# shacklettbp/madrona-learn

Hardware: AMD Instinct MI355X
Metric: env-steps/sec whole-node, 65536-env PPO, at 1/2/4/8 MI355X (higher is better)
Workload: dtype bf16; 1 GPU; 65536-env PPO iteration (BASELINE metric; SURVEY B8 semantics): T=32, obs=64, MLP[256,256], heads [4,8,5,5,2,2]+critic, 2 epochs x 32 minibatches of 2048 seqs (global), envs and minibatches split over 1 GPU(s); config=headline, total_envs=65536, envs_per_gpu=65536, global_minibatch_seqs=2048, minibatches_per_epoch=32, steps_per_update=32, parallelism=dp1, critic=scalar, hip_graph=True, sim_step=whole_rollout_one_launch

## Files before the change

### madrona-learn_amd/csrc/ppo_rows16.h

```cpp

#pragma once


template <int D> __device__ inline float r16_pair_dpp(float a, float b) {
    float r;
    if constexpr (D == 8)
        asm volatile(
            "s_nop 1\n\t"
            "v_add_f32_dpp %0, %1, %1 row_ror:8 row_mask:0xf bank_mask:0x3\n\t"
            "v_add_f32_dpp %0, %2, %2 row_ror:8 row_mask:0xf bank_mask:0xc"
            : "=&v"(r)
            : "v"(a), "v"(b));
    else
        asm volatile(
            "s_nop 1\n\t"
            "v_add_f32_dpp %0, %1, %1 row_ror:12 row_mask:0xf bank_mask:0x5\n\t"
            "v_add_f32_dpp %0, %2, %2 row_ror:4 row_mask:0xf bank_mask:0xa"
            : "=&v"(r)
            : "v"(a), "v"(b));
    return r;
}

__device__ inline int r16_colf(int qd, int lane) {
    const int r = lane & 15, g = lane >> 4;
    return 16 * (4 * qd + (r >> 2)) + 4 * g + (r & 3);
}
__device__ inline void r16_put_cols(float* cpl, const float (&cb)[4], const float (&cg)[4],
                                    int lane) {
#pragma unroll
    for (int qd = 0; qd < 4; ++qd) {
        const int f = r16_colf(qd, lane);
        cpl[f] = cb[qd];
        cpl[kR16H + f] = cg[qd];
    }
}

__device__ inline float r16_rowsum8(const float (&w)[8], int lane) {
    float x[4], y[2];
#pragma unroll
    for (int i = 0; i < 4; ++i) x[i] = r16_pair_dpp<4>(w[i], w[i + 4]);
    const bool h1 = (lane & 2) != 0, h0 = (lane & 1) != 0;
#pragma unroll
    for (int i = 0; i < 2; ++i) {
        const float keep = h1 ? x[i + 2] : x[i], send = h1 ? x[i] : x[i + 2];
        y[i] = keep + xlane<2>(send);
    }
    const float keep = h0 ? y[1] : y[0], send = h0 ? y[0] : y[1];
    return keep + xlane<1>(send);
}

__device__ inline float r16_dy(float z, float mean, float rstd, float gam, float bet, float da,
                               bool live, float& xh) {
    const float zc = z - mean;
    xh = zc * rstd;
    const float y = __builtin_fmaf(zc, rstd * gam, bet);
    return ((y > relu_thr<bf16>()) & live) ? da : 0.f;
}

__device__ inline void r16_dz_block(const f32x4& u, uint32_t (&zwb)[2], float mean,
                                    float rstd, float ca, float cbc, uint32_t (&dzb)[2]) {
#pragma unroll
    for (int k = 0; k < 2; ++k) {
        zwb[k] = r16_late(zwb[k]);
        const f2v zc = up_bf16(zwb[k]) - f2v{mean, mean};
        const f2v d = f2v{rstd, rstd} * f2v{u[2 * k], u[2 * k + 1]} +
                      (f2v{ca, ca} * zc + f2v{cbc, cbc});
        dzb[k] = pk_bf16(d.x, d.y);
    }
}

__device__ inline void r16_ln_bwd(f32x4 (&acc)[kR16NB], uint32_t (&zw)[kR16NB][2],
                                  float mean, float rstd, const float* gm, int g, int lane,
                                  bool live, uint32_t (&dzw)[kR16NB][2], float (&cb)[4],
                                  float (&cg)[4]) {
    mean = r16_late(mean);
    rstd = r16_late(rstd);
    float su = 0.f, sv = 0.f;
    constexpr int ord[4] = {0, 2, 1, 3};
    R16GB gb(gm, g, 0);
#pragma unroll
    for (int qd = 0; qd < kR16NB / 4; ++qd) {
        float wb[8], wg[8];
#pragma unroll
        for (int hp = 0; hp < 2; ++hp) {
            float pb[8], pg[8];
#pragma unroll
            for (int k = 0; k < 2; ++k) {
                const int step = 4 * qd + 2 * hp + k;
                const int b = 4 * qd + ord[2 * hp + k];
                float4 G, B;
                gb.take_now(b, G, B);
                const float gv[4] = {G.x, G.y, G.z, G.w}, bv[4] = {B.x, B.y, B.z, B.w};
                zw[b][0] = r16_late(zw[b][0]);
                zw[b][1] = r16_late(zw[b][1]);
#pragma unroll
                for (int i = 0; i < 4; ++i) {
                    float xh;
                    const float z = up_bf16(zw[b][i >> 1])[i & 1];
                    const float dy = r16_dy(z, mean, rstd, gv[i], bv[i], acc[b][i], live, xh);
                    const float u = dy * gv[i];
                    su += u;
                    sv = __builtin_fmaf(u, xh, sv);
                    acc[b][i] = u;
                    pb[4 * k + i] = dy;
                    pg[4 * k + i] = dy * xh;
                }
            }
            __builtin_amdgcn_sched_barrier(0);
#pragma unroll
            for (int i = 0; i < 4; ++i) {
                wb[4 * hp + i] = r16_pair_dpp<8>(pb[i], pb[4 + i]);
                wg[4 * hp + i] = r16_pair_dpp<8>(pg[i], pg[4 + i]);
            }
        }
        cb[qd] = r16_rowsum8(wb, lane);
        cg[qd] = r16_rowsum8(wg, lane);
    }
    su = add_xor32(add_xor16(su));
    sv = add_xor32(add_xor16(sv));
    const float invH = 1.0f / (float)kR16H;
    const float ca = -(rstd * rstd) * (sv * invH), cbc = -rstd * (su * invH);
#pragma unroll
    for (int b = 0; b < kR16NB; ++b) r16_dz_block(acc[b], zw[b], mean, rstd, ca, cbc, dzw[b]);
}

#ifdef ML_STAMPS
#define R16_STAMP(i) (r16_st[i] = __builtin_amdgcn_s_memtime())
#define R16_STAMPS_OUT()                                                              \
    do {                                                                              \
        if (ws.stamps && (tid & 63) == 0)                                             \
            for (int i_ = 0; i_ < 13; ++i_)                                           \
                ws.stamps[((int64_t)ptile * NT + tt) * 16 + i_] = r16_st[i_];        \
    } while (0)
#else
#define R16_STAMP(i) \
    do {             \
    } while (0)
#define R16_STAMPS_OUT() \
    do {                 \
    } while (0)
#endif

template <bool METRICS, int NW, int NT, int HC>
__global__ __launch_bounds__(64 * NW) __attribute__((amdgpu_waves_per_eu((NW + 3) / 4, (NW + 3) / 4))) void ppo_rows16_kernel(
    PolicyK P, RolloutK ro, const int32_t* __restrict__ mb_seq, int mb, int64_t M,
    const float* __restrict__ adv_st, HpK hp, WsK ws, R16Div dv) {
    extern __shared__ __attribute__((aligned(16))) char smem[];
#ifdef ML_STAMPS
    const uint64_t r16_t_entry = __builtin_amdgcn_s_memtime();
#endif
    typedef R16Lay<HC> LY;
    constexpr int LGS = LY::LGS, NHB = HC / 16;
    char* w1img = smem + LY::OffW1;
    char* whimg = smem + LY::OffWh;
    float* gb = (float*)(smem + LY::OffGb);
    float* hb = (float*)(smem + LY::OffHb);
    const float* bins = (const float*)(smem + LY::OffBins);
    const int tid = threadIdx.x;
    const int wave = __builtin_amdgcn_readfirstlane(tid >> 6);
    bf16* lgs = (bf16*)(smem + LY::OffLg) + wave * 16 * LGS;
    const int K = P.K;
    constexpr int D = kR16D, DS = D / 32;

    {
        static_assert(NW == kR16Waves, "r16_stage stages with kR16Waves waves");
        r16_stage<HC>(P, smem, tid);
        int* tab = (int*)(smem + LY::OffTab);
        if (tid <= MLEARN_MAX_GROUPS) {
            tab[tid] = P.off[tid];
            ((float*)tab)[MLEARN_MAX_GROUPS + 1 + tid] = tid < MLEARN_MAX_GROUPS ? hp.ecoef[tid] : 0.f;
            ((float*)tab)[2 * (MLEARN_MAX_GROUPS + 1) + tid] =
                tid < MLEARN_MAX_GROUPS ? hp.objw[tid] : 0.f;
        }
    }
    __syncthreads();
#ifdef ML_STAMPS
    const uint64_t r16_t_pro = __builtin_amdgcn_s_memtime();
#endif
    const int* t_off = (const int*)(smem + LY::OffTab);
    const float* t_ec = (const float*)t_off + MLEARN_MAX_GROUPS + 1;
    const float* t_ow = t_ec + MLEARN_MAX_GROUPS + 1;

    const int ptile = (int)blockIdx.x * NW + wave;
    const float as0 = adv_st[0], as1 = adv_st[1];
    VnVals vn{hp.norm_vals != 0, {0.f, 0.f, 0.f, 0.f}};
    if (hp.norm_vals)
        for (int i = 0; i < 4; ++i) vn.v[i] = adv_st[2 + i];
    LossAcc m;
    bool did = false;
    uint32_t dz0w[kR16NB][2];
    float cb0[4], cg0[4];
    float* prev_cp = nullptr;
    int64_t prev_row = -1;
    const int ntask = 16 * (K + 1);
    auto slot_of = [&](int64_t rw, uint32_t& tl) {
        const uint32_t f = (uint32_t)rw;
        tl = r16_udiv(f, dv.mb_mag, dv.mb_sh);
        return f - tl * (uint32_t)mb;
    };
    auto srow_of = [&](int64_t rw, uint32_t seq) -> int64_t {
        uint32_t tl;
        (void)slot_of(rw, tl);
        const uint32_t c = r16_udiv(seq, dv.n_mag, dv.n_sh), b = seq - c * (uint32_t)ro.N;
        return rw < M ? ((int64_t)c * ro.bptt + tl) * ro.ld + b : 0;
    };
    int64_t sr_n;
    {
        uint32_t tl;
        const int64_t rw = (int64_t)ptile * (16 * NT) + (tid & 15);
        sr_n = srow_of(rw, (uint32_t)mb_seq[slot_of(rw, tl)]);
    }

#pragma clang loop unroll(disable)
    for (int tt = 0; tt < NT; ++tt) {
#ifdef ML_STAMPS
        uint64_t r16_st[13];
#endif
        R16_STAMP(0);
        const int lane = r16_late(tid & 63), r = lane & 15, g = lane >> 4;
        const int64_t row0 = (int64_t)ptile * (16 * NT) + 16 * tt;
        const int64_t row = row0 + r;
        const bool live = row < M;
        const int64_t sr = sr_n;
        uint32_t seq_n = 0;
        if (tt + 1 < NT) {
            uint32_t tl;
            seq_n = (uint32_t)mb_seq[slot_of(row + 16, tl)];
        }
        bf16x8 xf[DS];
        const bf16* orow = (const bf16*)ro.obs + sr * D;
#pragma unroll
        for (int s = 0; s < DS; ++s)
            xf[s] = *(const bf16x8*)(orow + 32 * s + 8 * g);
        auto lda0 = [&](int ln) {
            const bf16* w0 = (const bf16*)P.wt[0];
            const int rr = ln & 15, gg = ln >> 4;
            return [=](int b, int s) {
                const int n = 16 * b + rr;
                const int64_t idx = ((int64_t)(((n >> 5) * (D >> 4) + 2 * s + (gg >> 1)) * 64 +
                                               (n & 31) + 32 * (gg & 1))) * 8;
                return *(const bf16x8*)(w0 + idx);
            };
        };
        const bool has_ret = ro.ret != nullptr, has_val = ro.values != nullptr;
        float t_adv = ro.adv[sr];
        float rv = (has_ret ? ro.ret : ro.adv)[sr], vv = (has_val ? ro.values : ro.adv)[sr];
        int ract[2];
        float rlp[2];
#pragma unroll
        for (int u = 0; u < 2; ++u) {
            const int grp = (lane + 64 * u) >> 4;
            const int ga = grp < K ? grp : K - 1;
            ract[u] = ro.actions[sr * K + ga];
            rlp[u] = ro.logp[sr * K + ga];
        }
        auto bf0 = [&](int s) { return xf[s]; };
        uint32_t zw0[kR16NB][2], zw[kR16NB][2], aw[kR16NB][2];
        float mean0, rstd0, mean, rstd;
        r16_fwd_layer<DS, kR16Ring0>(lda0(r16_late(lane)), bf0, zw0, mean0, rstd0);
        sr_n = srow_of(row + 16, r16_late(seq_n));
        uint32_t t_a[2];
        float t_b[2];
        {
            t_adv = r16_late(t_adv);
            rv = r16_late(rv);
            vv = r16_late(vv);
            const float retv = has_ret ? rv : t_adv + vv;
            const float ov = has_val ? vv : 0.f;
#pragma unroll
            for (int u = 0; u < 2; ++u) {
                const int grp = (lane + 64 * u) >> 4;
                t_a[u] = grp < K ? (uint32_t)r16_late(ract[u]) : __builtin_bit_cast(uint32_t, retv);
                t_b[u] = grp < K ? r16_late(rlp[u]) : ov;
            }
        }
        R16_STAMP(1);
#ifndef ML_PROBE_NO_X0
        {
            bf16* xrow = (bf16*)ws.x0 + r16_late(row) * D;
#pragma unroll
            for (int s = 0; s < DS; ++s)
                r16_st16(xrow + 32 * s + 8 * g, __builtin_bit_cast(u4r, xf[s]));
        }
#endif
        if (tt > 0) {
            r16_store_rows((bf16*)ws.dz[0] + r16_late(prev_row) * kR16H, dz0w, g);
            r16_put_cols(prev_cp, cb0, cg0, lane);
        }
        r16_ln_apply(zw0, mean0, rstd0, gb, g, aw);
        R16_STAMP(2);
        r16_fwd_layer<kR16KS, kR16Ring>(
            [&](int b, int s) { return r16_row_frag(w1img, 16 * b + r, s, g); },
            [&](int s) { return r16_bfrag(aw, s); }, zw, mean, rstd);
        R16_STAMP(3);
        if (NW > 4 && tt == 0 && wave >= NW / 2) __builtin_amdgcn_s_setprio(1);
#ifndef ML_PROBE_NO_A0
        r16_store_rows((bf16*)ws.a[0] + r16_late(row) * kR16H, aw, g);
#endif
        r16_ln_apply(zw, mean, rstd, gb + 2 * kR16H, g, aw);
        R16_STAMP(4);
        f32x4 ha[NHB];
#pragma unroll
        for (int j = 0; j < NHB; ++j) ha[j] = f32x4{0.f, 0.f, 0.f, 0.f};
        if constexpr (HC == 32) {
            r16_mm<NHB, kR16KS, 4>(
                ha, [&](int j, int s) { return r16_row_frag(whimg, 16 * j + r, s, g); },
                [&](int s) { return r16_bfrag(aw, s); });
        } else {
            const bf16* ht = (const bf16*)P.head_t;
            const uint32_t lo = r16_late((uint32_t)((r + 32 * (g & 1)) * 8 + 4 * (g >> 1)));
            r16_mm<NHB, kR16KS, kR16RingH>(
                ha,
                [&](int j, int s) {
                    const bf16* p = ht + ((j >> 1) * 8192 + s * 1024 + (j & 1) * 128);
                    const u2r a = *(const u2r*)(p + lo);
                    const u2r b = *(const u2r*)(p + 512 + lo);
                    return __builtin_bit_cast(bf16x8, u4r{a[0], a[1], b[0], b[1]});
                },
                [&](int s) { return r16_bfrag(aw, s); });
        }
        r16_store_rows((bf16*)ws.a[1] + r16_late(row) * kR16H, aw, g);
        {
            bf16* lr = lgs + r * LGS;
#pragma unroll
            for (int cbk = 0; cbk < NHB; ++cbk) {
                const int c0 = 16 * cbk + 4 * g;
                float v[4];
#pragma unroll
                for (int i = 0; i < 4; ++i) v[i] = rnd<bf16>(rnd<bf16>(ha[cbk][i]) + rnd<bf16>(hb[c0 + i]));
                *(u2r*)(lr + c0) = u2r{pk_bf16(v[0], v[1]), pk_bf16(v[2], v[3])};
            }
        }
        wave_lds_sync();
        R16_STAMP(5);
        auto loss_task = [&](int task, int act, float olp, float adv, float ret, float oval) {
            const int rr = task & 15, grp = task >> 4;
            bf16* lr = lgs + rr * LGS;
            if (row0 + rr >= M) {
                if (grp < K)
                    for (int j = t_off[grp]; j < t_off[grp + 1]; ++j) lr[j] = (bf16)0.f;
                else if (HC == 32)
                    for (int j = P.A; j < HC; ++j) lr[j] = (bf16)0.f;
                return;
            }
            if (grp < K) {
                if (hp.norm_adv) adv = (adv - as0) * as1;
                const int o0 = t_off[grp];
                loss_group(hp, lr + o0, t_off[grp + 1] - o0, act, olp, adv, t_ec[grp], t_ow[grp],
                           m);
            } else if (HC == 32) {
                loss_value(hp, lr, P.A, HC, ret, oval, m, vn);
            }
        };
        {
#pragma clang loop unroll(disable)
            for (int task = lane, u = 0; task < ntask; task += 64, ++u) {
                did = true;
                const uint32_t a = u == 0 ? t_a[0] : t_a[1];
                const float b = u == 0 ? t_b[0] : t_b[1];
                loss_task(task, (int)a, b, t_adv, __builtin_bit_cast(float, a), b);
            }
        }
        if constexpr (HC != 32) {
            wave_lds_sync();
            const uint32_t rbits = __shfl(K >= 4 ? t_a[1] : t_a[0], (16 * K + r) & 63);
            bf16* lr = lgs + r * LGS;
            const int CB = P.CB;
            if (row0 + r < M) {
                float mean;
                const float R = __builtin_bit_cast(float, rbits);
                const float vl = r16_twohot_ce(lr + P.A, CB, R, bins,
                                               hp.vcoef * hp.inv_s * hp.loss_scale, g, &mean);
                if (g == 0) {
                    const float verr = fabsf(mean - R);
                    m.svl += vl;
                    m.qvl += vl * vl;
                    m.mnvl = fminf(m.mnvl, vl);
                    m.mxvl = fmaxf(m.mxvl, vl);
                    m.serr += verr;
                    m.qerr += verr * verr;
                    m.mnerr = fminf(m.mnerr, verr);
                    m.mxerr = fmaxf(m.mxerr, verr);
                }
            } else {
                for (int j = P.A + g; j < P.A + CB; j += 4) lr[j] = (bf16)0.f;
            }
            for (int j = P.A + CB + g; j < HC; j += 4) lr[j] = (bf16)0.f;
        }
        wave_lds_sync();
        R16_STAMP(6);
        constexpr int HKS = HC / 32;
        bf16x8 dh[HKS];
#pragma unroll
        for (int s2 = 0; s2 < HKS; ++s2) {
            dh[s2] = *(const bf16x8*)(lgs + r * LGS + 32 * s2 + 8 * g);
            r16_st16((bf16*)ws.dhead + r16_late(row) * HC + 32 * s2 + 8 * g,
                     __builtin_bit_cast(u4r, dh[s2]));
        }
        float* cprow = ws.colpart + ((int64_t)ptile * NT + tt) * ws.CP;
#pragma unroll
        for (int c0 = 0; c0 < HC; c0 += 64) {
            if (c0 + lane < HC) {
                float hbs = 0.f;
#pragma unroll
                for (int rr = 0; rr < 16; ++rr) hbs += to_f32(lgs[rr * LGS + c0 + lane]);
                cprow[2 * 2 * kR16H + c0 + lane] = hbs;
            }
        }
        R16_STAMP(7);
        uint32_t dzw[kR16NB][2];
        {
            f32x4 hacc[kR16NB];
#pragma unroll
            for (int b = 0; b < kR16NB; ++b) hacc[b] = f32x4{0.f, 0.f, 0.f, 0.f};
            if constexpr (HC == 32) {
                r16_mm<kR16NB, 1, kR16Ring>(
                    hacc,
                    [&](int b, int) { return r16_tr_frag(whimg, 8 * g, 8 * g + 4, b, lane); },
                    [&](int) { return dh[0]; });
            } else {
                const bf16* hd = (const bf16*)P.head;
                const uint32_t lo = r16_late((uint32_t)((g >> 1) * 512 + (r + 32 * (g & 1)) * 8));
                r16_mm<kR16NB, HKS, kR16RingH>(
                    hacc,
                    [&](int b, int s2) {
                        const bf16* p = hd + ((b >> 1) * (HC / 16) * 512 + s2 * 1024 + (b & 1) * 128);
                        return *(const bf16x8*)(p + lo);
                    },
                    [&](int s2) { return dh[s2]; });
            }
            float cb1[4], cg1[4];
            r16_ln_bwd(hacc, zw, mean, rstd, gb + 2 * kR16H, g, lane, live, dzw, cb1, cg1);
            r16_put_cols(cprow + 2 * kR16H, cb1, cg1, lane);
        }
        r16_store_rows_keep((bf16*)ws.dz[1] + r16_late(row) * kR16H, dzw, g);
        R16_STAMP(8);
        f32x4 acc[kR16NB];
#pragma unroll
        for (int b = 0; b < kR16NB; ++b) acc[b] = f32x4{0.f, 0.f, 0.f, 0.f};
        r16_mm_bm<kR16NB, kR16KS, kR16Ring>(
            acc,
            [&](int b, int s) {
                return r16_tr_frag(w1img, 32 * s + 4 * g, 32 * s + 16 + 4 * g, b, lane);
            },
            [&](int s) { return r16_bfrag(dzw, s); });
        R16_STAMP(9);
        R16_STAMP(10);
        R16_STAMP(11);
        r16_ln_bwd(acc, zw0, mean0, rstd0, gb, g, lane, live, dz0w, cb0, cg0);
        prev_row = row;
        prev_cp = cprow;
        R16_STAMP(12);
        R16_STAMPS_OUT();
    }
    const int lane = tid & 63, r = lane & 15, g = lane >> 4;
    r16_store_rows((bf16*)ws.dz[0] + prev_row * kR16H, dz0w, g);
    r16_put_cols(prev_cp, cb0, cg0, lane);

#ifdef ML_STAMPS
    {
        __builtin_amdgcn_s_waitcnt(0);
        const uint64_t t_end = __builtin_amdgcn_s_memtime();
        if (ws.stamps && (tid & 63) == 0) {
            uint64_t* st = ws.stamps + (int64_t)ptile * NT * 16;
            st[13] = r16_t_entry;
            st[14] = r16_t_pro;
            st[15] = t_end;
        }
    }
#endif
    if (METRICS) {
        const float vals[kLossSlots] = {m.sobj, m.qobj, m.mnobj, m.mxobj, m.svl, m.qvl, m.mnvl,
                                        m.mxvl, m.serr, m.qerr, m.mnerr, m.mxerr, m.sent, m.qent,
                                        m.mnent, m.mxent, m.sentw, m.sobjw, 0.f, 0.f};
        constexpr int kUsed = 18;
        double* lp = ws.loss_part + (int64_t)ptile * kLossSlots;
        if (__any(did)) {
#pragma unroll
            for (int s = 0; s < kUsed; ++s) {
                const int kind = (s < 16) ? (s & 3) : 0;
                float v = vals[s];
                v = kind == 2 ? wave_reduce<2>(v) : (kind == 3 ? wave_reduce<3>(v) : wave_reduce<0>(v));
                if (lane == 0) lp[s] = v;
            }
            if (lane >= kUsed && lane < kLossSlots) lp[lane] = 0.0;
        } else if (lane < kLossSlots) {
            const int kind = (lane < 16) ? (lane & 3) : 0;
            lp[lane] = kind == 2 ? 3.4e38 : (kind == 3 ? -3.4e38 : 0.0);
        }
    }
}

struct R16Cfg {
    int nw, nt;
};
static R16Cfg rows16_cfg(int64_t Mp) {
    const int cus = device_cus();
    const int64_t kCUs = cus > 0 ? cus : 256;
    if (Mp % 256 == 0 && Mp / 256 >= kCUs) return R16Cfg{8, 2};
    if (Mp == 128 * kCUs) return R16Cfg{8, 1};
    return R16Cfg{0, 0};
}
static bool rows16_eligible(const PolicyK& P, int64_t Mp, int HC, int L, int H, bool bf) {
    const bool head = (HC == 32 && P.CB == 1) || (HC == 96 && P.CB > 1 && P.CB <= 64);
    return bf && H == kR16H && L == 2 && head && P.D == kR16D && P.K + 1 <= 8 &&
           rows16_cfg(Mp).nw > 0;
}

template <int NW, int NT, int HC>
static void launch_rows16_cfg(const PolicyK& P, const RolloutK& R, const int32_t* mb_seq, int mb,
                              int64_t M, const float* adv_st, const HpK& hp, const WsK& ws,
                              const R16Div& dv, hipStream_t s) {
    constexpr int lds = (int)R16Lay<HC>::Lds;
    if (set_lds_attr((const void*)ppo_rows16_kernel<true, NW, NT, HC>, lds, "ppo_rows16") ||
        set_lds_attr((const void*)ppo_rows16_kernel<false, NW, NT, HC>, lds, "ppo_rows16"))
        return;
    const int grid = (int)(ws.Mp / (16 * NW * NT));
    if (hp.metrics)
        hipLaunchKernelGGL((ppo_rows16_kernel<true, NW, NT, HC>), dim3(grid), dim3(64 * NW), lds,
                           s, P, R, mb_seq, mb, M, adv_st, hp, ws, dv);
    else
        hipLaunchKernelGGL((ppo_rows16_kernel<false, NW, NT, HC>), dim3(grid), dim3(64 * NW), lds,
                           s, P, R, mb_seq, mb, M, adv_st, hp, ws, dv);
}

static void launch_rows16(const PolicyK& P, const RolloutK& R, const int32_t* mb_seq, int mb,
                          int64_t M, const float* adv_st, const HpK& hp, const WsK& ws,
                          hipStream_t s) {
    R16Div dv;
    r16_magic((uint32_t)mb, dv.mb_mag, dv.mb_sh);
    r16_magic((uint32_t)R.N, dv.n_mag, dv.n_sh);
    const R16Cfg c = rows16_cfg(ws.Mp);
    if (P.HC == 32) {
        if (c.nt == 2)
            launch_rows16_cfg<8, 2, 32>(P, R, mb_seq, mb, M, adv_st, hp, ws, dv, s);
        else
            launch_rows16_cfg<8, 1, 32>(P, R, mb_seq, mb, M, adv_st, hp, ws, dv, s);
    } else {
        if (c.nt == 2)
            launch_rows16_cfg<8, 2, 96>(P, R, mb_seq, mb, M, adv_st, hp, ws, dv, s);
        else
            launch_rows16_cfg<8, 1, 96>(P, R, mb_seq, mb, M, adv_st, hp, ws, dv, s);
    }
}
```

### madrona-learn_amd/csrc/r16_common.h

```cpp
#pragma once

#include "common.h"
#include "dists.h"
#include "rowtile.h"

namespace ml {

constexpr int kR16Waves = 8;
constexpr int kR16Tiles = 2;
constexpr int kR16H = 256;
constexpr int kR16NB = kR16H / 16;
constexpr int kR16KS = kR16H / 32;
constexpr int kR16HC = MLEARN_HEAD_COLS;
constexpr int kR16D = 64;
constexpr int kR16LGS = 40;
#ifndef ML_R16_RING
#define ML_R16_RING 6
#endif
#ifndef ML_R16_RING0
#define ML_R16_RING0 16
#endif
constexpr int kR16Ring = ML_R16_RING;
constexpr int kR16Ring0 = ML_R16_RING0;
#ifndef ML_R16_RINGH
#define ML_R16_RINGH 8
#endif
constexpr int kR16RingH = ML_R16_RINGH;
constexpr int kR16TabN = 3 * (MLEARN_MAX_GROUPS + 1);
template <int HC> struct R16Lay {
    static_assert(HC == 32 || HC == 96, "head width");
    static constexpr int LGS = HC == 32 ? kR16LGS : 104;
    static constexpr size_t OffW1 = 0;
    static constexpr size_t OffWh = OffW1 + (size_t)kR16H * 512;
    static constexpr size_t OffGb = OffWh + (HC == 32 ? (size_t)HC * 512 : 0);
    static constexpr size_t OffHb = OffGb + (size_t)2 * 2 * kR16H * 4;
    static constexpr size_t OffBins = OffHb + (size_t)HC * 4;
    static constexpr size_t OffLg = OffBins + (HC == 32 ? 0 : (size_t)64 * 4);
    static constexpr size_t OffTab = OffLg + (size_t)kR16Waves * 16 * LGS * 2;
    static constexpr size_t Lds = OffTab + (size_t)kR16TabN * 4;
    static_assert(Lds <= 160 * 1024, "row-split LDS budget");
};

typedef float f2v __attribute__((ext_vector_type(2)));
typedef short short4r __attribute__((ext_vector_type(4)));
typedef __attribute__((ext_vector_type(4))) uint32_t u4r;
typedef __attribute__((ext_vector_type(2))) uint32_t u2r;

__device__ inline uint32_t r16_off(int n, int u) {
    const int sw = ((n & 7) << 2) | (((n >> 3) & 1) << 1);
    return (uint32_t)(n * 512 + ((u ^ sw) << 3));
}

template <typename V> __device__ inline V r16_late(V v) {
    asm volatile("" : "+v"(v));
    return v;
}

__device__ inline f32x4 mma16(bf16x8 a, bf16x8 b, f32x4 c) {
    return __builtin_amdgcn_mfma_f32_16x16x32_bf16(a, b, c, 0, 0, 0);
}

__device__ inline bf16x8 r16_row_frag(const char* img, int n, int s, int g) {
    const u2r lo = *(const u2r*)(img + r16_off(n, 8 * s + g));
    const u2r hi = *(const u2r*)(img + r16_off(n, 8 * s + 4 + g));
    const u4r v = {lo[0], lo[1], hi[0], hi[1]};
    return __builtin_bit_cast(bf16x8, v);
}

__device__ inline bf16x8 r16_tr_frag(const char* img, int rlo, int rhi, int b, int lane) {
    const int q = (lane >> 2) & 3, p = lane & 3;
    typedef __attribute__((address_space(3))) short4r* lp;
    const short4r lo = __builtin_amdgcn_ds_read_tr16_b64_v4i16(
        (lp)(img + (rlo & ~15) * 512 + r16_off((rlo & 15) + q, 4 * b + p)));
    const short4r hi = __builtin_amdgcn_ds_read_tr16_b64_v4i16(
        (lp)(img + (rhi & ~15) * 512 + r16_off((rhi & 15) + q, 4 * b + p)));
    typedef short short8r __attribute__((ext_vector_type(8)));
    const short8r v = {lo[0], lo[1], lo[2], lo[3], hi[0], hi[1], hi[2], hi[3]};
    return __builtin_bit_cast(bf16x8, v);
}

__device__ inline void r16_st16(void* p, u4r v) { *(u4r*)p = v; }

__device__ inline uint32_t pk_bf16(float a, float b) {
    typedef __bf16 bf16x2 __attribute__((ext_vector_type(2)));
    const bf16x2 v = {(bf16)a, (bf16)b};
    return __builtin_bit_cast(uint32_t, v);
}
__device__ inline f2v up_bf16(uint32_t w) {
    return f2v{__builtin_bit_cast(float, w << 16), __builtin_bit_cast(float, w & 0xffff0000u)};
}
__device__ inline bf16x8 r16_bfrag(const uint32_t (&w)[kR16NB][2], int s) {
    const u4r v = {w[2 * s][0], w[2 * s][1], w[2 * s + 1][0], w[2 * s + 1][1]};
    return __builtin_bit_cast(bf16x8, v);
}

template <int NBO, int NS, int RING, typename LDA, typename BF>
__device__ inline void r16_mm(f32x4 (&acc)[NBO], LDA lda, BF bfrag) {
    constexpr int N = NS * NBO;
    constexpr int RG = RING < N ? RING : N;
    __builtin_amdgcn_sched_barrier(0);
    bf16x8 ra[RG];
#pragma unroll
    for (int i = 0; i < RG; ++i) ra[i] = lda(i % NBO, i / NBO);
    bf16x8 bfr = bfrag(0);
#pragma unroll
    for (int i = 0; i < N; ++i) {
        const bf16x8 a = ra[i % RG];
        if (i + RG < N) ra[i % RG] = lda((i + RG) % NBO, (i + RG) / NBO);
        __builtin_amdgcn_sched_barrier(0);
        acc[i % NBO] = mma16(a, bfr, acc[i % NBO]);
        __builtin_amdgcn_sched_barrier(0);
        if ((i + 1) % NBO == 0 && i + 1 < N) bfr = bfrag((i + 1) / NBO);
    }
}

template <int NBO, int NS, int RING, typename LDA, typename BF>
__device__ inline void r16_mm_bm(f32x4 (&acc)[NBO], LDA lda, BF bfrag) {
    static_assert(NBO % 2 == 0, "block pairs");
    constexpr int N = NS * NBO;
    constexpr int RG = RING < N ? RING : N;
    auto jof = [](int i) { return 2 * (i / (2 * NS)) + (i & 1); };
    auto sof = [](int i) { return (i >> 1) % NS; };
    __builtin_amdgcn_sched_barrier(0);
    bf16x8 ra[RG];
#pragma unroll
    for (int i = 0; i < RG; ++i) ra[i] = lda(jof(i), sof(i));
#pragma unroll
    for (int i = 0; i < N; ++i) {
        const bf16x8 a = ra[i % RG];
        if (i + RG < N) ra[i % RG] = lda(jof(i + RG), sof(i + RG));
        __builtin_amdgcn_sched_barrier(0);
        acc[jof(i)] = mma16(a, bfrag(sof(i)), acc[jof(i)]);
        __builtin_amdgcn_sched_barrier(0);
    }
}

template <int NS, int RING, typename LDA, typename BF>
__device__ inline void r16_fwd_layer(LDA lda, BF bfrag, uint32_t (&zw)[kR16NB][2], float& mean_o,
                                     float& rstd_o) {
    f2v s2 = {0.f, 0.f}, q2 = {0.f, 0.f};
#pragma unroll
    for (int h = 0; h < 2; ++h) {
        f32x4 acc[8];
#pragma unroll
        for (int j = 0; j < 8; ++j) acc[j] = f32x4{0.f, 0.f, 0.f, 0.f};
        r16_mm<8, NS, RING>(acc, [&](int j, int s) { return lda(8 * h + j, s); }, bfrag);
#pragma unroll
        for (int j = 0; j < 8; ++j)
#pragma unroll
            for (int k = 0; k < 2; ++k) {
                zw[8 * h + j][k] = pk_bf16(acc[j][2 * k], acc[j][2 * k + 1]);
                const f2v x = up_bf16(zw[8 * h + j][k]);
                s2 += x;
                q2 = x * x + q2;
            }
    }
    float sum = s2.x + s2.y, sq = q2.x + q2.y;
    sum = add_xor32(add_xor16(sum));
    sq = add_xor32(add_xor16(sq));
    const float invH = 1.0f / (float)kR16H;
    const float mean = sum * invH;
    const float var = fmaxf(sq * invH - mean * mean, 0.f);
    mean_o = mean;
    rstd_o = rsqrtf(var + 1e-6f);
}

__device__ inline void r16_store_rows(bf16* rowp, uint32_t (&w)[kR16NB][2], int g) {
#pragma unroll
    for (int c = 0; c < kR16NB / 2; ++c) {
#pragma unroll
        for (int k = 0; k < 2; ++k) {
            const auto v = __builtin_amdgcn_permlane16_swap(w[2 * c][k], w[2 * c + 1][k], false,
                                                            false);
            w[2 * c][k] = v[0];
            w[2 * c + 1][k] = v[1];
        }
        const int blk = 2 * c + (g & 1);
        r16_st16(rowp + 16 * blk + 8 * (g >> 1),
                 u4r{w[2 * c][0], w[2 * c][1], w[2 * c + 1][0], w[2 * c + 1][1]});
    }
}

__device__ inline void r16_store_rows_keep(bf16* rowp, const uint32_t (&w)[kR16NB][2], int g) {
#pragma unroll
    for (int c = 0; c < kR16NB / 2; ++c) {
        uint32_t t[2][2];
#pragma unroll
        for (int k = 0; k < 2; ++k) {
            const auto v = __builtin_amdgcn_permlane16_swap(w[2 * c][k], w[2 * c + 1][k], false,
                                                            false);
            t[0][k] = v[0];
            t[1][k] = v[1];
        }
        const int blk = 2 * c + (g & 1);
        r16_st16(rowp + 16 * blk + 8 * (g >> 1), u4r{t[0][0], t[0][1], t[1][0], t[1][1]});
    }
}

struct R16GB {
    const float* gm;
    int g;
    float4 G, B;
    __device__ R16GB(const float* gm_, int g_, int first) : gm(gm_), g(g_) { load(first); }
    __device__ void load(int b) {
        const int f0 = r16_late(16 * b + 4 * g);
        G = *(const float4*)(gm + f0);
        B = *(const float4*)(gm + kR16H + f0);
    }
    __device__ void take_now(int b, float4& Go, float4& Bo) {
        __builtin_amdgcn_sched_barrier(0);
        load(b);
        Go = G;
        Bo = B;
    }
    __device__ void take(int following, float4& Go, float4& Bo) {
        __builtin_amdgcn_sched_barrier(0);
        Go = G;
        Bo = B;
        if (following >= 0) load(following);
    }
};

__device__ inline void r16_ln_apply(uint32_t (&zw)[kR16NB][2], float mean, float rstd,
                                    const float* gm, int g, uint32_t (&aw)[kR16NB][2]) {
    const f2v m2 = {mean, mean}, r2 = {rstd, rstd};
    R16GB gb(gm, g, 0);
#pragma unroll
    for (int b = 0; b < kR16NB; ++b) {
        float4 G, B;
        gb.take(b + 1 < kR16NB ? b + 1 : -1, G, B);
        zw[b][0] = r16_late(zw[b][0]);
        zw[b][1] = r16_late(zw[b][1]);
        const f2v y0 = __builtin_elementwise_fma(up_bf16(zw[b][0]) - m2, r2 * f2v{G.x, G.y},
                                                 f2v{B.x, B.y});
        const f2v y1 = __builtin_elementwise_fma(up_bf16(zw[b][1]) - m2, r2 * f2v{G.z, G.w},
                                                 f2v{B.z, B.w});
        aw[b][0] = pk_bf16(fmaxf(y0.x, 0.f), fmaxf(y0.y, 0.f));
        aw[b][1] = pk_bf16(fmaxf(y1.x, 0.f), fmaxf(y1.y, 0.f));
    }
}

struct R16Div {
    uint32_t mb_mag, n_mag;
    int mb_sh, n_sh;
};
__device__ inline uint32_t r16_udiv(uint32_t n, uint32_t mag, int sh) {
    return (__umulhi(n, mag) + n) >> sh;
}


template <int HC = kR16HC>
__device__ inline void r16_stage(const PolicyK& P, char* smem, int tid) {
    typedef R16Lay<HC> LY;
    char* w1img = smem + LY::OffW1;
    char* whimg = smem + LY::OffWh;
    float* gb = (float*)(smem + LY::OffGb);
    float* hb = (float*)(smem + LY::OffHb);
    {
        const u4r* src1 = (const u4r*)P.wt[1];
        const u4r* srch = (const u4r*)P.head_t;
        constexpr int N1 = kR16H * kR16H * 2 / 16 / (64 * kR16Waves);
        u4r v1[N1], vh[2];
#pragma unroll
        for (int i = 0; i < N1; ++i) v1[i] = src1[tid + i * 64 * kR16Waves];
        if (HC == 32)
#pragma unroll
            for (int i = 0; i < 2; ++i) vh[i] = srch[tid + i * 64 * kR16Waves];
        float pv[2];
#pragma unroll
        for (int i = 0; i < 2; ++i) {
            const int j = tid + i * 64 * kR16Waves, l = j >> 9, c = j & 511;
            pv[i] = c < kR16H ? P.lns[l][c] : P.lnb[l][c - kR16H];
        }
        const float hbv = tid < HC ? P.head_b[tid] : 0.f;
        auto put = [&](char* img, int U, u4r v) {
            const int n = ((U >> 10) << 5) | (U & 31), h = (U >> 5) & 1, s16 = (U >> 6) & 15;
            *(u2r*)(img + r16_off(n, 4 * s16 + h)) = u2r{v[0], v[1]};
            *(u2r*)(img + r16_off(n, 4 * s16 + 2 + h)) = u2r{v[2], v[3]};
        };
#pragma unroll
        for (int i = 0; i < N1; ++i) put(w1img, tid + i * 64 * kR16Waves, v1[i]);
        if (HC == 32)
#pragma unroll
            for (int i = 0; i < 2; ++i) put(whimg, tid + i * 64 * kR16Waves, vh[i]);
#pragma unroll
        for (int i = 0; i < 2; ++i) gb[tid + i * 64 * kR16Waves] = pv[i];
        if (tid < HC) hb[tid] = hbv;
        if (HC != 32 && tid < P.CB)
            ((float*)(smem + LY::OffBins))[tid] = twohot_bin(tid, P.CB);
    }
}

__device__ inline bf16x8 r16_head_l2(const bf16* head_t, int n, int s, int g) {
    const int64_t base =
        ((int64_t)(((n >> 5) * 16 + 2 * s) * 64 + (n & 31) + 32 * (g & 1))) * 8 + 4 * (g >> 1);
    const u2r lo = *(const u2r*)(head_t + base);
    const u2r hi = *(const u2r*)(head_t + base + 512);
    const u4r v = {lo[0], lo[1], hi[0], hi[1]};
    return __builtin_bit_cast(bf16x8, v);
}

__device__ inline float r16_twohot_ce(bf16* lr, int CB, float R, const float* bins, float scale,
                                      int g, float* mean_out) {
    float cle = 0.f, cgt = 0.f;
    for (int j = g; j < CB; j += 4) {
        cle += bins[j] <= R ? 1.f : 0.f;
        cgt += bins[j] > R ? 1.f : 0.f;
    }
    cle += __shfl_xor(cle, 16);
    cle += __shfl_xor(cle, 32);
    cgt += __shfl_xor(cgt, 16);
    cgt += __shfl_xor(cgt, 32);
    const int lo = min(max((int)cle - 1, 0), CB - 1);
    const int up = min(max(CB - (int)cgt, 0), CB - 1);
    const bool same = lo == up;
    const float dl = same ? 1.f : fabsf(bins[lo] - R);
    const float du = same ? 1.f : fabsf(bins[up] - R);
    const float tot = dl + du;
    const float wl = dl / tot, wu = du / tot;
    float mx = -3.4e38f;
    for (int j = g; j < CB; j += 4) mx = fmaxf(mx, to_f32(lr[j]));
    mx = fmaxf(mx, __shfl_xor(mx, 16));
    mx = fmaxf(mx, __shfl_xor(mx, 32));
    float se = 0.f;
    for (int j = g; j < CB; j += 4) se += __expf(to_f32(lr[j]) - mx);
    se += __shfl_xor(se, 16);
    se += __shfl_xor(se, 32);
    const int mid = (CB - 1) / 2;
    float acc = 0.f;
    for (int i = g; i < mid; i += 4) {
        const int a = mid - 1 - i, b = mid + 1 + i;
        acc += (__expf(to_f32(lr[a]) - mx) / se) * bins[a] +
               (__expf(to_f32(lr[b]) - mx) / se) * bins[b];
    }
    acc += __shfl_xor(acc, 16);
    acc += __shfl_xor(acc, 32);
    *mean_out = (__expf(to_f32(lr[mid]) - mx) / se) * bins[mid] + acc;
    const float lse = mx + __logf(se);
    const float llo = to_f32(lr[lo]), lup = to_f32(lr[up]);
    const float loss = -(wl * (llo - lse) + wu * (lup - lse));
    const float wsum = wl + wu;
    for (int j = g; j < CB; j += 4) {
        const float pj = __expf(to_f32(lr[j]) - mx) / se;
        const float w = (j == lo ? wl : 0.f) + (j == up ? wu : 0.f);
        lr[j] = (bf16)((wsum * pj - w) * scale);
    }
    return loss;
}

__device__ inline float r16_twohot_mean(const bf16* lr, int CB, const float* bins, int g) {
    float mx = -3.4e38f;
    for (int j = g; j < CB; j += 4) mx = fmaxf(mx, to_f32(lr[j]));
    mx = fmaxf(mx, __shfl_xor(mx, 16));
    mx = fmaxf(mx, __shfl_xor(mx, 32));
    float se = 0.f;
    for (int j = g; j < CB; j += 4) se += __expf(to_f32(lr[j]) - mx);
    se += __shfl_xor(se, 16);
    se += __shfl_xor(se, 32);
    const int mid = (CB - 1) / 2;
    float acc = 0.f;
    for (int i = g; i < mid; i += 4) {
        const int a = mid - 1 - i, b = mid + 1 + i;
        acc += (__expf(to_f32(lr[a]) - mx) / se) * bins[a] +
               (__expf(to_f32(lr[b]) - mx) / se) * bins[b];
    }
    acc += __shfl_xor(acc, 16);
    acc += __shfl_xor(acc, 32);
    return (__expf(to_f32(lr[mid]) - mx) / se) * bins[mid] + acc;
}

static inline void r16_magic(uint32_t d, uint32_t& mag, int& sh) {
    int l = 0;
    while ((1ull << l) < d) ++l;
    mag = (uint32_t)(((1ull << 32) * ((1ull << l) - d)) / d + 1);
    sh = l;
}

}
```

Measured before the change: 232.6 million env-steps/s.

## Prefetch next row tile's rollout inputs and overlap first gather with weight staging

Gathering of observations, advantages, returns, values, actions and log-probs moves into a load_in helper that fills a register struct. The first tile's gather is issued in the prologue, interleaved with the global loads of the weight images and parameters before they are written to LDS. With METRICS off, each iteration loads the next tile's inputs early, after the dz store, so global latency overlaps the backward matmul. This raises register pressure and leaves compile-time switches for alternative placement.

```diff
diff --git a/madrona-learn_amd/csrc/ppo_rows16.h b/madrona-learn_amd/csrc/ppo_rows16.h
--- a/madrona-learn_amd/csrc/ppo_rows16.h
+++ b/madrona-learn_amd/csrc/ppo_rows16.h
@@ -141,6 +141,13 @@
     } while (0)
 #endif
 
+template <int DS> struct R16In {
+    bf16x8 xf[DS];
+    float adv, rv, vv;
+    int act[2];
+    float lp[2];
+};
+
 template <bool METRICS, int NW, int NT, int HC>
 __global__ __launch_bounds__(64 * NW) __attribute__((amdgpu_waves_per_eu((NW + 3) / 4, (NW + 3) / 4))) void ppo_rows16_kernel(
     PolicyK P, RolloutK ro, const int32_t* __restrict__ mb_seq, int mb, int64_t M,
@@ -162,37 +169,7 @@
     const int K = P.K;
     constexpr int D = kR16D, DS = D / 32;
 
-    {
-        static_assert(NW == kR16Waves, "r16_stage stages with kR16Waves waves");
-        r16_stage<HC>(P, smem, tid);
-        int* tab = (int*)(smem + LY::OffTab);
-        if (tid <= MLEARN_MAX_GROUPS) {
-            tab[tid] = P.off[tid];
-            ((float*)tab)[MLEARN_MAX_GROUPS + 1 + tid] = tid < MLEARN_MAX_GROUPS ? hp.ecoef[tid] : 0.f;
-            ((float*)tab)[2 * (MLEARN_MAX_GROUPS + 1) + tid] =
-                tid < MLEARN_MAX_GROUPS ? hp.objw[tid] : 0.f;
-        }
-    }
-    __syncthreads();
-#ifdef ML_STAMPS
-    const uint64_t r16_t_pro = __builtin_amdgcn_s_memtime();
-#endif
-    const int* t_off = (const int*)(smem + LY::OffTab);
-    const float* t_ec = (const float*)t_off + MLEARN_MAX_GROUPS + 1;
-    const float* t_ow = t_ec + MLEARN_MAX_GROUPS + 1;
-
     const int ptile = (int)blockIdx.x * NW + wave;
-    const float as0 = adv_st[0], as1 = adv_st[1];
-    VnVals vn{hp.norm_vals != 0, {0.f, 0.f, 0.f, 0.f}};
-    if (hp.norm_vals)
-        for (int i = 0; i < 4; ++i) vn.v[i] = adv_st[2 + i];
-    LossAcc m;
-    bool did = false;
-    uint32_t dz0w[kR16NB][2];
-    float cb0[4], cg0[4];
-    float* prev_cp = nullptr;
-    int64_t prev_row = -1;
-    const int ntask = 16 * (K + 1);
     auto slot_of = [&](int64_t rw, uint32_t& tl) {
         const uint32_t f = (uint32_t)rw;
         tl = r16_udiv(f, dv.mb_mag, dv.mb_sh);
@@ -204,12 +181,78 @@
         const uint32_t c = r16_udiv(seq, dv.n_mag, dv.n_sh), b = seq - c * (uint32_t)ro.N;
         return rw < M ? ((int64_t)c * ro.bptt + tl) * ro.ld + b : 0;
     };
-    int64_t sr_n;
+    const bool has_ret = ro.ret != nullptr, has_val = ro.values != nullptr;
+    auto load_in = [&](int64_t sr, int ln, R16In<DS>& in) {
+        const bf16* orow = (const bf16*)ro.obs + sr * D;
+#pragma unroll
+        for (int s = 0; s < DS; ++s)
+            in.xf[s] = *(const bf16x8*)(orow + 32 * s + 8 * (ln >> 4));
+        in.adv = ro.adv[sr];
+        in.rv = (has_ret ? ro.ret : ro.adv)[sr];
+        in.vv = (has_val ? ro.values : ro.adv)[sr];
+#pragma unroll
+        for (int u = 0; u < 2; ++u) {
+            const int grp = (ln + 64 * u) >> 4;
+            const int ga = grp < K ? grp : K - 1;
+            in.act[u] = ro.actions[sr * K + ga];
+            in.lp[u] = ro.logp[sr * K + ga];
+        }
+    };
+    static_assert(NW == kR16Waves, "R16Stage stages with kR16Waves waves");
+    R16In<DS> in;
     {
         uint32_t tl;
         const int64_t rw = (int64_t)ptile * (16 * NT) + (tid & 15);
-        sr_n = srow_of(rw, (uint32_t)mb_seq[slot_of(rw, tl)]);
-    }
+        R16Stage<HC> stg;
+        int tb_off = 0;
+        float tb_ec = 0.f, tb_ow = 0.f;
+#ifdef ML_R16_GATHER_FIRST
+        load_in(srow_of(rw, (uint32_t)mb_seq[slot_of(rw, tl)]), tid & 63, in);
+#else
+        const uint32_t seq0 = (uint32_t)mb_seq[slot_of(rw, tl)];
+#endif
+        __builtin_amdgcn_sched_barrier(0);
+        if (tid <= MLEARN_MAX_GROUPS) {
+            tb_off = P.off[tid];
+            tb_ec = tid < MLEARN_MAX_GROUPS ? hp.ecoef[tid] : 0.f;
+            tb_ow = tid < MLEARN_MAX_GROUPS ? hp.objw[tid] : 0.f;
+        }
+        stg.load_params(P, tid);
+        stg.load_images(P, tid);
+#ifndef ML_R16_GATHER_FIRST
+        __builtin_amdgcn_sched_barrier(0);
+        load_in(srow_of(rw, r16_late(seq0)), tid & 63, in);
+        __builtin_amdgcn_sched_barrier(0);
+#endif
+        stg.put(P, smem, tid);
+        int* tab = (int*)(smem + LY::OffTab);
+        if (tid <= MLEARN_MAX_GROUPS) {
+            tab[tid] = tb_off;
+            ((float*)tab)[MLEARN_MAX_GROUPS + 1 + tid] = tb_ec;
+            ((float*)tab)[2 * (MLEARN_MAX_GROUPS + 1) + tid] = tb_ow;
+        }
+    }
+    const float as0 = adv_st[0], as1 = adv_st[1];
+    VnVals vn{hp.norm_vals != 0, {0.f, 0.f, 0.f, 0.f}};
+    if (hp.norm_vals)
+        for (int i = 0; i < 4; ++i) vn.v[i] = adv_st[2 + i];
+    __syncthreads();
+#ifdef ML_STAMPS
+    const uint64_t r16_t_pro = __builtin_amdgcn_s_memtime();
+#endif
+    const int* t_off = (const int*)(smem + LY::OffTab);
+    const float* t_ec = (const float*)t_off + MLEARN_MAX_GROUPS + 1;
+    const float* t_ow = t_ec + MLEARN_MAX_GROUPS + 1;
+
+    LossAcc m;
+    bool did = false;
+    uint32_t dz0w[kR16NB][2];
+    float cb0[4], cg0[4];
+    float* prev_cp = nullptr;
+    int64_t prev_row = -1;
+    const int ntask = 16 * (K + 1);
+    int64_t sr_n = 0;
+    constexpr bool kAhead = !METRICS;
 
 #pragma clang loop unroll(disable)
     for (int tt = 0; tt < NT; ++tt) {
@@ -221,17 +264,32 @@
         const int64_t row0 = (int64_t)ptile * (16 * NT) + 16 * tt;
         const int64_t row = row0 + r;
         const bool live = row < M;
-        const int64_t sr = sr_n;
+        if (kAhead || tt == 0) {
+#pragma unroll
+            for (int s = 0; s < DS; ++s)
+                in.xf[s] = __builtin_bit_cast(bf16x8, r16_late(__builtin_bit_cast(u4r, in.xf[s])));
+            in.adv = r16_late(in.adv);
+            in.rv = r16_late(in.rv);
+            in.vv = r16_late(in.vv);
+#pragma unroll
+            for (int u = 0; u < 2; ++u) {
+                in.act[u] = r16_late(in.act[u]);
+                in.lp[u] = r16_late(in.lp[u]);
+            }
+        } else {
+            load_in(sr_n, lane, in);
+        }
+        bf16x8 xf[DS];
+#pragma unroll
+        for (int s = 0; s < DS; ++s) xf[s] = in.xf[s];
+        float t_adv = in.adv, rv = in.rv, vv = in.vv;
+        int ract[2] = {in.act[0], in.act[1]};
+        float rlp[2] = {in.lp[0], in.lp[1]};
         uint32_t seq_n = 0;
         if (tt + 1 < NT) {
             uint32_t tl;
             seq_n = (uint32_t)mb_seq[slot_of(row + 16, tl)];
         }
-        bf16x8 xf[DS];
-        const bf16* orow = (const bf16*)ro.obs + sr * D;
-#pragma unroll
-        for (int s = 0; s < DS; ++s)
-            xf[s] = *(const bf16x8*)(orow + 32 * s + 8 * g);
         auto lda0 = [&](int ln) {
             const bf16* w0 = (const bf16*)P.wt[0];
             const int rr = ln & 15, gg = ln >> 4;
@@ -242,18 +300,6 @@
                 return *(const bf16x8*)(w0 + idx);
             };
         };
-        const bool has_ret = ro.ret != nullptr, has_val = ro.values != nullptr;
-        float t_adv = ro.adv[sr];
-        float rv = (has_ret ? ro.ret : ro.adv)[sr], vv = (has_val ? ro.values : ro.adv)[sr];
-        int ract[2];
-        float rlp[2];
-#pragma unroll
-        for (int u = 0; u < 2; ++u) {
-            const int grp = (lane + 64 * u) >> 4;
-            const int ga = grp < K ? grp : K - 1;
-            ract[u] = ro.actions[sr * K + ga];
-            rlp[u] = ro.logp[sr * K + ga];
-        }
         auto bf0 = [&](int s) { return xf[s]; };
         uint32_t zw0[kR16NB][2], zw[kR16NB][2], aw[kR16NB][2];
         float mean0, rstd0, mean, rstd;
@@ -434,6 +480,15 @@
             r16_put_cols(cprow + 2 * kR16H, cb1, cg1, lane);
         }
         r16_store_rows_keep((bf16*)ws.dz[1] + r16_late(row) * kR16H, dzw, g);
+#ifndef ML_R16_AHEAD_LATE
+        if (kAhead && tt + 1 < NT) {
+            __builtin_amdgcn_sched_barrier(0);
+            load_in(r16_late(sr_n), lane, in);
+            __builtin_amdgcn_sched_barrier(0);
+        } else {
+            in = R16In<DS>{};
+        }
+#endif
         R16_STAMP(8);
         f32x4 acc[kR16NB];
 #pragma unroll
@@ -445,6 +500,15 @@
             },
             [&](int s) { return r16_bfrag(dzw, s); });
         R16_STAMP(9);
+#ifdef ML_R16_AHEAD_LATE
+        if (kAhead && tt + 1 < NT) {
+            __builtin_amdgcn_sched_barrier(0);
+            load_in(r16_late(sr_n), lane, in);
+            __builtin_amdgcn_sched_barrier(0);
+        } else {
+            in = R16In<DS>{};
+        }
+#endif
         R16_STAMP(10);
         R16_STAMP(11);
         r16_ln_bwd(acc, zw0, mean0, rstd0, gb, g, lane, live, dz0w, cb0, cg0);
diff --git a/madrona-learn_amd/csrc/r16_common.h b/madrona-learn_amd/csrc/r16_common.h
--- a/madrona-learn_amd/csrc/r16_common.h
+++ b/madrona-learn_amd/csrc/r16_common.h
@@ -249,46 +249,56 @@
 }
 
 
-template <int HC = kR16HC>
-__device__ inline void r16_stage(const PolicyK& P, char* smem, int tid) {
+template <int HC = kR16HC> struct R16Stage {
     typedef R16Lay<HC> LY;
-    char* w1img = smem + LY::OffW1;
-    char* whimg = smem + LY::OffWh;
-    float* gb = (float*)(smem + LY::OffGb);
-    float* hb = (float*)(smem + LY::OffHb);
-    {
+    static constexpr int N1 = kR16H * kR16H * 2 / 16 / (64 * kR16Waves);
+    u4r v1[N1], vh[2];
+    float pv[2], hbv;
+    __device__ inline void load_images(const PolicyK& P, int tid) {
         const u4r* src1 = (const u4r*)P.wt[1];
         const u4r* srch = (const u4r*)P.head_t;
-        constexpr int N1 = kR16H * kR16H * 2 / 16 / (64 * kR16Waves);
-        u4r v1[N1], vh[2];
 #pragma unroll
         for (int i = 0; i < N1; ++i) v1[i] = src1[tid + i * 64 * kR16Waves];
         if (HC == 32)
 #pragma unroll
             for (int i = 0; i < 2; ++i) vh[i] = srch[tid + i * 64 * kR16Waves];
-        float pv[2];
+    }
+    __device__ inline void load_params(const PolicyK& P, int tid) {
 #pragma unroll
         for (int i = 0; i < 2; ++i) {
             const int j = tid + i * 64 * kR16Waves, l = j >> 9, c = j & 511;
             pv[i] = c < kR16H ? P.lns[l][c] : P.lnb[l][c - kR16H];
         }
-        const float hbv = tid < HC ? P.head_b[tid] : 0.f;
-        auto put = [&](char* img, int U, u4r v) {
+        hbv = tid < HC ? P.head_b[tid] : 0.f;
+    }
+    __device__ inline void put(const PolicyK& P, char* smem, int tid) const {
+        char* w1img = smem + LY::OffW1;
+        char* whimg = smem + LY::OffWh;
+        float* gb = (float*)(smem + LY::OffGb);
+        float* hb = (float*)(smem + LY::OffHb);
+        auto put1 = [&](char* img, int U, u4r v) {
             const int n = ((U >> 10) << 5) | (U & 31), h = (U >> 5) & 1, s16 = (U >> 6) & 15;
             *(u2r*)(img + r16_off(n, 4 * s16 + h)) = u2r{v[0], v[1]};
             *(u2r*)(img + r16_off(n, 4 * s16 + 2 + h)) = u2r{v[2], v[3]};
         };
 #pragma unroll
-        for (int i = 0; i < N1; ++i) put(w1img, tid + i * 64 * kR16Waves, v1[i]);
+        for (int i = 0; i < N1; ++i) put1(w1img, tid + i * 64 * kR16Waves, v1[i]);
         if (HC == 32)
 #pragma unroll
-            for (int i = 0; i < 2; ++i) put(whimg, tid + i * 64 * kR16Waves, vh[i]);
+            for (int i = 0; i < 2; ++i) put1(whimg, tid + i * 64 * kR16Waves, vh[i]);
 #pragma unroll
         for (int i = 0; i < 2; ++i) gb[tid + i * 64 * kR16Waves] = pv[i];
         if (tid < HC) hb[tid] = hbv;
         if (HC != 32 && tid < P.CB)
             ((float*)(smem + LY::OffBins))[tid] = twohot_bin(tid, P.CB);
     }
+};
+template <int HC = kR16HC>
+__device__ inline void r16_stage(const PolicyK& P, char* smem, int tid) {
+    R16Stage<HC> st;
+    st.load_images(P, tid);
+    st.load_params(P, tid);
+    st.put(P, smem, tid);
 }
 
 __device__ inline bf16x8 r16_head_l2(const bf16* head_t, int n, int s, int g) {
```

Measured after the change: 243.9 million env-steps/s (median of 6 runs). +4.9%, better.
